# DillionLowry/NeuralCodecs

Hardware: AMD Instinct MI355X
Metric: audio-seconds/sec encode+decode (x real-time), DAC-44.1kHz B=32 (higher is better)
Workload: dtype f32; 1 GPU; DAC 44.1kHz 8kbps encode+decode, batch=32 x 1 s clips per GPU (BASELINE configs[1]); clips_per_gpu=32, global_batch=32, collective=none

## Files before the change

### neuralcodecs_amd/csrc/nc_conv_small.hip

```cpp
#include <cstdlib>
#include <type_traits>
#include <utility>
#include <vector>

#include "nc_conv.h"
#include "nc_frag.h"
#include "nc_gn.h"
#include "nc_math.h"

namespace nc {

typedef float small_f32x4 __attribute__((ext_vector_type(4)));

constexpr int SMALL_CB = 8;
constexpr int SMALL_PF = 12;

struct ConvSmallArgs {
    const float* x;
    int64_t x_bstride, x_cstride;
    int x_len;
    int in_left, in_Lz, in_L;
    const float* in_stats; const float* in_gamma; const float* in_beta; int in_elu;
    double* gn_part; int gn_nrb, gn_ncb; unsigned* gn_count; float* gn_stats; double gn_n;
    const float* wp;
    const float* bias;
    const float* alpha_out;
    float* y;
    int64_t y_bstride, y_cstride;
    int Cin, Cout, K, stride, pad, dil, Tout;
    int n_t_tiles, n_row_tiles;
    int W;
    int groups;
};

__device__ __forceinline__ float small_epilogue(const ConvSmallArgs& a, int row, float v) {
    v = v + (a.bias ? a.bias[row] : 0.0f);
    if (a.alpha_out) {
        const float al = a.alpha_out[row];
        v = nc_snakef(v, al, nc_snake_inv(al));
    }
    return v;
}

__global__ __launch_bounds__(256) void conv_small_kernel(const ConvSmallArgs a) {
    extern __shared__ __attribute__((aligned(16))) float xs[];
    const int tid = threadIdx.x, lane = tid & 63;
    const int wave = __builtin_amdgcn_readfirstlane(tid >> 6);
    int bid = blockIdx.x;
    const int rt = bid % a.n_row_tiles; bid /= a.n_row_tiles;
    const int tt = bid % a.n_t_tiles;
    const int b = bid / a.n_t_tiles;
    const int K = a.K, W = a.W, dil = a.dil;
    const int col = lane & 15, kq = lane >> 4;
    const int g0 = tt * 16 * a.stride - a.pad;
    const float* xb = a.x + (int64_t)b * a.x_bstride;
    const small_f32x4* wsrc = reinterpret_cast<const small_f32x4*>(a.wp) + ((int64_t)(4 * rt + wave) * a.groups) * 64 + lane;
    const int groups = a.groups;
    small_f32x4 ring[SMALL_PF];
#pragma unroll
    for (int i = 0; i < SMALL_PF; ++i) ring[i] = wsrc[(int64_t)min(i, groups - 1) * 64];
    const int n_blocks = (a.Cin + SMALL_CB - 1) / SMALL_CB;
    const int n_slots = SMALL_CB * W;
    constexpr int NS = 6;
    float rx[NS];
    auto issue = [&](int cbk) __attribute__((always_inline)) {
#pragma unroll
        for (int u = 0; u < NS; ++u) {
            const int i = tid + 256 * u;
            const int c = i / W, j = i - c * W;
            const int ci = cbk * SMALL_CB + c;
            int g = g0 + j;
            bool ok = (i < n_slots) & (ci < a.Cin) & (g >= 0) & (g < a.x_len);
            if (a.in_L > 0) {
                int q = g - a.in_left;
                q = q < 0 ? -q : q;
                if (q >= a.in_Lz) q = 2 * (a.in_Lz - 1) - q;
                ok = ok & (q >= 0) & (q < a.in_L);
                g = q;
            }
            rx[u] = ok ? xb[(int64_t)ci * a.x_cstride + g] : 0.0f;
        }
    };
    auto store = [&](float* dst) __attribute__((always_inline)) {
#pragma unroll
        for (int u = 0; u < NS; ++u) {
            const int i = tid + 256 * u;
            if (i < n_slots) dst[i] = rx[u];
        }
    };
    issue(0);
    store(xs);
    __syncthreads();
    small_f32x4 acc = {0.0f, 0.0f, 0.0f, 0.0f};
    const int groups_per_block = SMALL_CB * K / 16;
    int cbk = 0, gblk = 0;
    const float* xc = xs;
    if (n_blocks > 1) issue(1);
    int k = kq, off = col * a.stride + kq * dil;
    auto read_group = [&](float (&bv)[4]) __attribute__((always_inline)) {
#pragma unroll
        for (int j = 0; j < 4; ++j) {
            bv[j] = xc[off];
            k += 4; off += 4 * dil;
            if (k >= K) { k -= K; off += W - K * dil; }
        }
    };
    float bc[4], bn[4];
    read_group(bc);
    for (int gbase = 0; gbase < groups; gbase += SMALL_PF) {
        nc_static_for<SMALL_PF>([&](auto it) __attribute__((always_inline)) {
            constexpr int i = decltype(it)::value;
            if (gbase + i < groups) {
                const small_f32x4 wv = ring[i];
                ring[i] = wsrc[(int64_t)min(gbase + i + SMALL_PF, groups - 1) * 64];
                const bool last_of_block = gblk + 1 == groups_per_block;
                if (!last_of_block) read_group(bn);
#pragma unroll
                for (int j = 0; j < 4; ++j) acc = __builtin_amdgcn_mfma_f32_16x16x4f32(wv[j], bc[j], acc, 0, 0, 0);
                if (last_of_block) {
                    ++cbk;
                    gblk = 0;
                    if (cbk < n_blocks) {
                        store(xs + (cbk & 1) * n_slots);
                        __syncthreads();
                        xc = xs + (cbk & 1) * n_slots;
                        if (cbk + 1 < n_blocks) issue(cbk + 1);
                        k = kq; off = col * a.stride + kq * dil;
                        read_group(bn);
                    }
                } else {
                    ++gblk;
                }
#pragma unroll
                for (int j = 0; j < 4; ++j) bc[j] = bn[j];
            }
        });
    }
    const int t = tt * 16 + col;
    if (t < a.Tout) {
        float* yb = a.y + (int64_t)b * a.y_bstride + t;
#pragma unroll
        for (int r = 0; r < 4; ++r) {
            const int row = (4 * rt + wave) * 16 + 4 * kq + r;
            if (row < a.Cout) yb[(int64_t)row * a.y_cstride] = small_epilogue(a, row, acc[r]);
        }
    }
}

template <int GPB, int NB, int TN = 1, int CB = SMALL_CB, int NS = (TN == 1 ? 6 : TN == 2 ? 9 : 18), bool INM = false, bool GN = false>
__global__ __launch_bounds__(256) void conv_small_unrolled_kernel(const ConvSmallArgs a) {
    constexpr int BNC = 16 * TN;
    constexpr int PF = GPB * NB;
    extern __shared__ __attribute__((aligned(16))) float xs[];
    const int tid = threadIdx.x, lane = tid & 63;
    const int wave = __builtin_amdgcn_readfirstlane(tid >> 6);
    int bid = blockIdx.x;
    const int rt = bid % a.n_row_tiles; bid /= a.n_row_tiles;
    const int tt = bid % a.n_t_tiles;
    const int b = bid / a.n_t_tiles;
    const int K = a.K, W = a.W, dil = a.dil;
    const int col = lane & 15, kq = lane >> 4;
    const int g0 = tt * BNC * a.stride - a.pad;
    const float* xb = a.x + (int64_t)b * a.x_bstride;
    const small_f32x4* wsrc = reinterpret_cast<const small_f32x4*>(a.wp) + ((int64_t)(4 * rt + wave) * a.groups) * 64 + lane;
    const int groups = a.groups;
    small_f32x4 ring[PF];
#pragma unroll
    for (int i = 0; i < PF; ++i) ring[i] = wsrc[(int64_t)min(i, groups - 1) * 64];
    const int n_blocks = a.Cin / CB;
    const int n_slots = CB * W;
    float rx[NS];
    float2* const Gt = reinterpret_cast<float2*>(xs + 2 * n_slots);
    float in_mu = 0.0f, in_rs = 1.0f;
    if constexpr (INM) {
        if (a.in_stats) {
            in_mu = a.in_stats[2 * b]; in_rs = a.in_stats[2 * b + 1];
            for (int i = tid; i < a.Cin; i += 256) Gt[i] = make_float2(a.in_gamma[i], a.in_beta[i]);
        }
        __syncthreads();
    }
    int xo[NS], cu[INM ? NS : 1];
    unsigned okm = 0;
#pragma unroll
    for (int u = 0; u < NS; ++u) {
        const int i = tid + 256 * u;
        const int c = i / W, j = i - c * W;
        if constexpr (INM) cu[u] = min(c, CB - 1);
        int g = g0 + j;
        bool ok = (i < n_slots) & (g >= 0) & (g < a.x_len);
        if (a.in_L > 0) {
            int q = g - a.in_left;
            q = q < 0 ? -q : q;
            if (q >= a.in_Lz) q = 2 * (a.in_Lz - 1) - q;
            ok = ok & (q >= 0) & (q < a.in_L);
            g = q;
        }
        if (ok) okm |= 1u << u;
        xo[u] = ok ? c * (int)a.x_cstride + g : 0;
    }
    auto issue = [&](int cbk) __attribute__((always_inline)) {
        const float* xr = xb + (int64_t)cbk * CB * a.x_cstride;
#pragma unroll
        for (int u = 0; u < NS; ++u) rx[u] = xr[xo[u]];
    };
    auto store = [&](float* dst, int cbk) __attribute__((always_inline)) {
#pragma unroll
        for (int u = 0; u < NS; ++u) {
            const int i = tid + 256 * u;
            float v = rx[u];
            if constexpr (INM) {
                if (a.in_stats) {
                    const float2 gb = Gt[cbk * CB + cu[u]];
                    v = ((v - in_mu) * in_rs) * gb.x + gb.y;
                }
                if (a.in_elu) v = nc_eluf(v);
            }
            if (i < n_slots) dst[i] = ((okm >> u) & 1u) ? v : 0.0f;
        }
    };
    issue(0);
    store(xs, 0);
    __syncthreads();
    small_f32x4 acc[TN];
#pragma unroll
    for (int c = 0; c < TN; ++c) acc[c] = small_f32x4{0.0f, 0.0f, 0.0f, 0.0f};
    const int off0 = col * a.stride + kq * dil, cts = 16 * a.stride;
    for (int cb0 = 0; cb0 < n_blocks; cb0 += NB) {
        nc_static_for<NB>([&](auto bt) __attribute__((always_inline)) {
            constexpr int nb = decltype(bt)::value;
            const int cbk = cb0 + nb;
            const float* xc = xs + (cbk & 1) * n_slots;
            const int nxt = min(cbk + 1, n_blocks - 1);
            issue(nxt);
            int k = kq, off = off0;
            if constexpr (CB == 64) { k = 0; off = col * a.stride + kq * W; }
            else if (k >= K) { k -= K; off += W - K * dil; }
            float bv[2][4][TN];
            auto read_group = [&](float (&v)[4][TN]) __attribute__((always_inline)) {
#pragma unroll
                for (int j = 0; j < 4; ++j) {
#pragma unroll
                    for (int c = 0; c < TN; ++c) v[j][c] = xc[off + c * cts];
                    if constexpr (CB == 64) {
                        off += 4 * W;
                    } else {
                        k += 4; off += 4 * dil;
                        if (k >= K) { k -= K; off += W - K * dil; }
                        if (k >= K) { k -= K; off += W - K * dil; }
                    }
                }
            };
            read_group(bv[0]);
            nc_static_for<GPB>([&](auto gt) __attribute__((always_inline)) {
                constexpr int g = decltype(gt)::value, ri = nb * GPB + g;
                const small_f32x4 wv = ring[ri];
                ring[ri] = wsrc[(int64_t)min((cbk + NB) * GPB + g, groups - 1) * 64];
                if constexpr (g + 1 < GPB) read_group(bv[(g + 1) & 1]);
#pragma unroll
                for (int j = 0; j < 4; ++j)
#pragma unroll
                    for (int c = 0; c < TN; ++c) acc[c] = __builtin_amdgcn_mfma_f32_16x16x4f32(wv[j], bv[g & 1][j][c], acc[c], 0, 0, 0);
            });
            store(xs + ((cbk + 1) & 1) * n_slots, nxt);
            __syncthreads();
        });
    }
    if constexpr (GN) {
        static_assert(!GN || TN == 2, "the GroupNorm epilogue reduces whole 32x32 blocks: 32-column tiles");
        float* const tile = xs;
#pragma unroll
        for (int c = 0; c < TN; ++c)
#pragma unroll
            for (int r = 0; r < 4; ++r) {
                const int lr = 16 * wave + 4 * kq + r, row = 64 * rt + lr;
                tile[lr * 33 + c * 16 + col] = acc[c][r] + ((a.bias && row < a.Cout) ? a.bias[row] : 0.0f);
            }
        __syncthreads();
        if (wave < 2) {
            const int h = lane >> 5, cc = lane & 31;
            const int t = tt * 32 + cc;
            float vv[16];
            unsigned okm16 = 0;
#pragma unroll
            for (int r = 0; r < 16; ++r) {
                const int lr = 32 * wave + (r & 3) + 8 * (r >> 2) + 4 * h;
                vv[r] = tile[lr * 33 + cc];
                if ((64 * rt + lr < a.Cout) & (t < a.Tout)) okm16 |= 1u << r;
            }
            double s1, s2;
            nc_gn_slot_sums<false>(vv, okm16, s1, s2);
            nc_gn_butterfly(s1, s2);
            const int rbk = 2 * rt + wave, cbk = tt;
            if (lane == 0 && rbk < a.gn_nrb && cbk < a.gn_ncb)
                nc_gn_store_partial(a.gn_part + (((int64_t)b * a.gn_nrb + rbk) * a.gn_ncb + cbk) * 2, s1, s2);
        }
        if (a.gn_count != nullptr)
            nc_gn_arrive_and_finish(a.gn_part + (int64_t)b * a.gn_nrb * a.gn_ncb * 2, a.gn_count + b, a.gn_stats + 2 * b, a.gn_nrb * a.gn_ncb,
                                    (unsigned)(a.n_row_tiles * a.n_t_tiles), a.gn_n);
    }
#pragma unroll
    for (int c = 0; c < TN; ++c) {
        const int t = tt * BNC + c * 16 + col;
        if (t < a.Tout) {
            float* yb = a.y + (int64_t)b * a.y_bstride + t;
#pragma unroll
            for (int r = 0; r < 4; ++r) {
                const int row = (4 * rt + wave) * 16 + 4 * kq + r;
                if (row < a.Cout) yb[(int64_t)row * a.y_cstride] = small_epilogue(a, row, acc[c][r]);
            }
        }
    }
}

void pack_conv_small(const float* dense_w, int Cin, int Cout, int K, std::vector<float>& out) {
    const int tiles = ((Cout + 63) / 64) * 4, groups = Cin * K / 16;
    out.assign((size_t)tiles * groups * 256, 0.0f);
    for (int tile = 0; tile < tiles; ++tile)
        for (int g = 0; g < groups; ++g)
            for (int l = 0; l < 64; ++l)
                for (int j = 0; j < 4; ++j) {
                    const int row = 16 * tile + (l & 15), kk = 16 * g + 4 * j + (l >> 4);
                    if (row < Cout) out[(((size_t)tile * groups + g) * 64 + l) * 4 + j] = dense_w[(size_t)row * Cin * K + kk];
                }
}

static bool small_k1(int Cin, int Cout, int K, int stride) { return K == 1 && stride == 1 && Cin % 256 == 0 && Cout >= 1024; }
static bool small_k7(int Cin, int K, int stride, int dil) { return (K == 7 || K == 3) && stride == 1 && dil == 1 && Cin % 32 == 0; }

bool conv_small_eligible(int Cin, int Cout, int K, int stride, int dil, bool transposed) {
    if (!transposed && small_k1(Cin, Cout, K, stride)) return true;
    if (!transposed && Cout >= 64 && small_k7(Cin, K, stride, dil)) return true;
    if (transposed || K < 4 || stride < 2 || Cout < 64) return false;
    if ((Cin * K) % 16 != 0 || (SMALL_CB * K) % 16 != 0 || Cin % SMALL_CB != 0) return false;
    const int W = 15 * stride + (K - 1) * dil + 1;
    return SMALL_CB * W <= 6 * 256 && (size_t)2 * SMALL_CB * W * 4 <= 64 * 1024;
}

int conv_small_max_tn(int Cin, int K, int stride, int dil) {
    if (K == 1 && stride == 1 && Cin % 256 == 0) return 2;
    if (small_k7(Cin, K, stride, dil)) return 2;
    const int W32 = 31 * stride + (K - 1) * dil + 1;
    const bool k16 = K * SMALL_CB / 16 == 8 && Cin % SMALL_CB == 0 && (Cin / SMALL_CB) % 2 == 0;
    return (k16 && SMALL_CB * W32 <= 9 * 256) ? 2 : 1;
}

bool conv_small_gn_available(int Cin, int K, int stride, int dil, bool inm) {
    if (conv_small_max_tn(Cin, K, stride, dil) < 2) return false;
    if (small_k7(Cin, K, stride, dil)) return K == 3 ? Cin <= 1024 : !inm;
    return !inm;
}

bool conv_small_inm_available(int Cin, int K, int stride, int dil) { return K == 3 && small_k7(Cin, K, stride, dil) && Cin <= 1024; }

bool launch_conv_small(const float* x, int64_t x_bstride, int64_t x_cstride, int x_len, int in_left, int in_Lz, int in_L, const float* in_stats,
                       const float* in_gamma, const float* in_beta, int in_elu, const ConvSmallGn* gn, const float* wp, const float* bias, const float* alpha_out, float* y,
                       int64_t y_bstride, int64_t y_cstride, int B, int Cin, int Cout, int K, int stride, int pad, int dil, int Tout, int want_tn, hipStream_t s) {
    ConvSmallArgs a{};
    a.x = x; a.x_bstride = x_bstride; a.x_cstride = x_cstride; a.x_len = x_len; a.wp = wp; a.bias = bias; a.alpha_out = alpha_out;
    a.in_left = in_left; a.in_Lz = in_Lz; a.in_L = in_L;
    a.in_stats = in_stats; a.in_gamma = in_gamma; a.in_beta = in_beta; a.in_elu = in_elu;
    if (gn && gn->part) {
        if (alpha_out || conv_small_max_tn(Cin, K, stride, dil) < 2) return false;
        a.gn_part = gn->part; a.gn_nrb = gn->nrb; a.gn_ncb = gn->ncb; a.gn_count = gn->count; a.gn_stats = gn->stats; a.gn_n = gn->n;
        want_tn = 2;
    }
    const bool with_gn = a.gn_part != nullptr;
    const bool inm = in_stats != nullptr || in_elu != 0;
    if (inm && !conv_small_inm_available(Cin, K, stride, dil)) return false;
    a.y = y; a.y_bstride = y_bstride; a.y_cstride = y_cstride;
    a.Cin = Cin; a.Cout = Cout; a.K = K; a.stride = stride; a.pad = pad; a.dil = dil; a.Tout = Tout;
    a.n_row_tiles = (Cout + 63) / 64;
    a.groups = Cin * K / 16;
    static const int tn_env = (int)env_int("NC_SMALL_TN", 0);
    const int W64 = 63 * stride + (K - 1) * dil + 1;
    const bool tn2_fits = conv_small_max_tn(Cin, K, stride, dil) >= 2, tn4_fits = tn2_fits && SMALL_CB * W64 <= 18 * 256;
    const int TN = with_gn ? 2 : (tn4_fits && tn_env == 4 && !small_k7(Cin, K, stride, dil)) ? 4 : (tn2_fits && (tn_env == 2 || (tn_env == 0 && want_tn >= 2))) ? 2 : 1;
    a.n_t_tiles = (Tout + 16 * TN - 1) / (16 * TN);
    a.W = (16 * TN - 1) * stride + (K - 1) * dil + 1;
    const bool k7 = small_k7(Cin, K, stride, dil), k1 = small_k1(Cin, Cout, K, stride);
    size_t lds = (size_t)2 * (k1 ? 64 : k7 ? 16 : SMALL_CB) * a.W * sizeof(float) + (inm ? (size_t)Cin * sizeof(float2) : 0);
    if (with_gn) lds = std::max(lds, (size_t)64 * 33 * sizeof(float));
    const int64_t grid = (int64_t)B * a.n_t_tiles * a.n_row_tiles;
    if (grid <= 0 || grid > 0x7fffffff) return false;
    static const bool rolled_only = env_flag("NC_SMALL_ROLLED");
    const int gpb = SMALL_CB * K / 16, n_blocks = Cin / SMALL_CB;
    const bool fits31 = (int64_t)Cin * x_cstride + x_len < ((int64_t)1 << 31);
    void (*fn)(const ConvSmallArgs) = conv_small_kernel;
    if (k1) {
        if (!fits31 || TN != 2 || with_gn || inm) return false;
        fn = conv_small_unrolled_kernel<4, 4, 2, 64, 8>;
    } else if (k7) {
        if (!fits31) return false;
        if (with_gn) {
            if (K == 7 && !inm) fn = conv_small_unrolled_kernel<7, 2, 2, 16, 3, false, true>;
            else if (K == 3) fn = conv_small_unrolled_kernel<3, 2, 2, 16, 3, true, true>;
            else return false;
        } else if (K == 7) fn = TN == 2 ? conv_small_unrolled_kernel<7, 2, 2, 16, 3> : conv_small_unrolled_kernel<7, 2, 1, 16, 2>;
        else if (inm) fn = TN == 2 ? conv_small_unrolled_kernel<3, 2, 2, 16, 3, true> : conv_small_unrolled_kernel<3, 2, 1, 16, 2, true>;
        else fn = TN == 2 ? conv_small_unrolled_kernel<3, 2, 2, 16, 3> : conv_small_unrolled_kernel<3, 2, 1, 16, 2>;
    } else if (TN == 4) {
        if (!fits31) return false;
        fn = conv_small_unrolled_kernel<8, 2, 4>;
    } else if (TN == 2) {
        if (!fits31 || (with_gn && inm)) return false;
        fn = with_gn ? conv_small_unrolled_kernel<8, 2, 2, SMALL_CB, 9, false, true> : conv_small_unrolled_kernel<8, 2, 2>;
    } else if (!rolled_only && fits31 && Cin % SMALL_CB == 0) {
        if (gpb == 8 && n_blocks % 2 == 0) fn = conv_small_unrolled_kernel<8, 2>;
        else if (gpb == 4 && n_blocks % 4 == 0) fn = conv_small_unrolled_kernel<4, 4>;
        else if (gpb == 5 && n_blocks % 4 == 0) fn = conv_small_unrolled_kernel<5, 4>;
        else if (gpb == 3 && n_blocks % 6 == 0) fn = conv_small_unrolled_kernel<3, 6>;
        else if (gpb == 2 && n_blocks % 8 == 0) fn = conv_small_unrolled_kernel<2, 8>;
    }
    hipLaunchKernelGGL(fn, dim3((unsigned)grid), dim3(256), lds, s, a);
    NC_HIP(hipGetLastError());
    return true;
}

}
```

### neuralcodecs_amd/csrc/nc_util.hip

```cpp
#include <cmath>
#include <mutex>
#include <set>
#include <tuple>

#include "nc_common.h"
#include "nc_model.h"

namespace nc {

static thread_local std::string g_last_error;
void set_last_error(const char* msg) { g_last_error = msg ? msg : ""; }
const char* get_last_error() { return g_last_error.c_str(); }

namespace {
struct EnvRow { const char* name; char kind; const char* doc; };
const EnvRow kEnv[] = {
    {"NC_NO_FLAT", 'b', "one-clip column tiles instead of the flattened (clip, column) axis"},
    {"NC_NO_FLAT_GN", 'b', "one-clip tiles wherever GroupNorm sums are emitted"},
    {"NC_CO_GROUP", 'i', "cap of the row-tile groups (1 = one weight panel per XCD)"},
    {"NC_NO_WIDE_FUSE", 'b', "no whole-channel fused residual units (C = 256)"},
    {"NC_WIDE_FUSE_192", 'b', "whole-channel fused unit at C = 192 as well"},
    {"NC_NO_FUSE", 'b', "every residual unit in two launches"},
    {"NC_NO_TILE_ALTS", 'b', "primary row-tile height only"},
    {"NC_TM_PICK", 'i', "force a packed row-tile variant"},
    {"NC_TM_FORCE", 'i', "force the row-tile height where it divides Cout"},
    {"NC_TN_THRESH", 'i', "column-tile width threshold"},
    {"NC_NO_TN_ROUNDS", 'b', "no round-count rule for the column-tile width"},
    {"NC_NO_XR", 'b', "generic B-fragment addressing in the conv template (no constant-pitch immediate offsets)"},
    {"NC_NO_XV", 'b', "legacy instances with item-wise window staging everywhere (no XV-only instances)"},
    {"NC_XV_K7_MIN_COLS", 'i', "columns per clip from which the k = 7 convolutions take the XV-only instances (0: wherever the rows are 64-byte aligned)"},
    {"NC_NO_XV_K7", 'b', "legacy instances for the k = 7 residual-unit convolutions (no XV-only instances on the long rows)"},
    {"NC_NO_NARROW", 'b', "no 3-wave narrow variants"},
    {"NC_NO_SLIM", 'b', "no half-size reduction blocks for narrow long rows"},
    {"NC_NO_SUBPIXEL", 'b', "per-phase launches for power-of-two strided transposed convolutions"},
    {"NC_NO_SUBPIXEL_ANY", 'b', "per-phase launches for the other strides (3, 5)"},
    {"NC_NO_CONV1X1", 'b', "pointwise layers through the windowed template"},
    {"NC_NO_SKINNY", 'b', "no skinny projection kernel (Cout <= 16)"},
    {"NC_NO_THIN", 'b', "PCM heads through the matrix-core template"},
    {"NC_THIN_NO_VEC", 'p', "scalar window loads in the thin-output kernel"},
    {"NC_NO_THIN_INM", 'b', "summed copy + plain head instead of the input-mode head"},
    {"NC_NO_STEM", 'b', "stems through the matrix-core template"},
    {"NC_NO_TINY_TILES", 'b', "no smallest-tile rule for tiny grids"},
    {"NC_TINY_BLOCKS", 'i', "grid size below which the tiny-grid rule applies (256)"},
    {"NC_NO_DIST_SMALL", 'b', "segmented staging on small grids"},
    {"NC_DIST_MAX_GRID", 'i', "largest grid that takes distributed staging (768)"},
    {"NC_NO_CONV_SMALL", 'b', "no short-row 16x16x4 kernel"},
    {"NC_SMALL_MAX_GRID", 'i', "largest short-row grid (2048)"},
    {"NC_SMALL_WIDE_BELOW", 'i', "template grid below which the 32-column short-row form is taken (512)"},
    {"NC_SMALL_K1_COLS", 'i', "columns up to which k = 1 layers take the short-row kernel (4096; 0 = off)"},
    {"NC_SMALL_TN", 'i', "force the short-row column tiles (1 | 2 | 4)"},
    {"NC_SMALL_ROLLED", 'b', "rolled short-row loop"},
    {"NC_DAC_RVQ_STAGEWISE", 'p', "DAC quantizer stage by stage"},
    {"NC_EUCLID_NO_MFMA", 'p', "vector Euclidean codebook search"},
    {"NC_ENCODEC_NO_FUSE", 'b', "padded / activated copies instead of the fused SConv1d input mode"},
    {"NC_ENCODEC_NO_OVERLAP", 'b', "segment groups one after the other"},
    {"NC_NO_GN_FUSE", 'b', "stand-alone GroupNorm sums"},
    {"NC_NO_GN_FINISH", 'b', "separate GroupNorm final launch"},
    {"NC_NO_IN2", 'b', "summed copies instead of the two-input staging mode"},
    {"NC_NO_CONV3S", 'b', "windowed k = 3 instead of the streaming kernel"},
    {"NC_DAC_PITCH", 'b', "DAC activation rows at pitch L rounded up to 16 samples (64-byte aligned rows: the 696-step layers take the XV-only instances; measured slower)"},
    {"NC_NO_DOWN2", 'b', "Encodec 48 kHz encoder: the windowed two-input instance for the stride-2 down-convolution instead of the streaming kernel"},
    {"NC_NO_DOWN4", 'b', "Encodec 48 kHz encoder: summed copy + windowed instance for the stride-4 down-convolution instead of the streaming kernel"},
    {"NC_NO_DOWN5", 'b', "Encodec 48 kHz encoder: summed copy + windowed instance for the stride-5 down-convolution instead of the streaming kernel"},
    {"NC_NO_UP_PITCH", 'b', "Encodec transposed convolutions write dense rows (the trimmed view of the stride-5 layer then starts on an odd sample)"},
    {"NC_NO_UP4", 'b', "Encodec 48 kHz decoder: summed copy + windowed instance for the stride-4 up-convolution instead of the streaming kernel"},
    {"NC_NO_UP2", 'b', "Encodec 48 kHz decoder: the windowed two-input instance for the stride-2 up-convolution instead of the streaming kernel"},
    {"NC_RMS_TWO_PASS", 'b', "Encodec RMS scale as two launches (chunk sums, final) instead of the one-launch form"},
    {"NC_NO_RES_A", 'b', "residual blocks of the Encodec 48 kHz outer stages: shortcut and k = 3 branch as two launches instead of the fused first pass"},
    {"NC_SYNC_ACQUIRE", 'b', "agent-scope acquire fence behind the persistent LSTM's flag poll and in front of the in-launch GroupNorm finish"},
    {"NC_LSTM_STEPWISE", 'b', "one LSTM launch per step"},
    {"NC_LSTM_CHUNKS", 'i', "layer-pipeline chunks of the per-layer persistent LSTM (6; 1 = layers in sequence)"},
    {"NC_LSTM_EVEN_CHUNKS", 'b', "equal LSTM chunks"},
    {"NC_LSTM_UB", 'i', "hidden-unit blocks per LSTM workgroup (2 | 4)"},
    {"NC_LSTM_NO_HTILE", 'b', "persistent LSTM: every wavefront fetches its own h operands, W_hh in LDS (the form before the LDS h tile)"},
    {"NC_LSTM_NO_ELU", 'b', "the consumer applies the ELU behind an SLSTM"},
    {"NC_LSTM_FAKE_TIMEOUT", 'b', "tests: report the first persistent LSTM launch as timed out"},
    {"NC_SNAC_NO_FUSE", 'b', "SNAC residual units in two launches (depthwise, pointwise)"},
    {"NC_SNAC_FUSE_MIN_COLS", 'i', "columns (clips x steps) from which the one-launch SNAC residual unit is taken (65536)"},
    {"NC_SNAC_FUSE_MAX_ELEMS", 'i', "channels x steps of ONE clip up to which the one-launch SNAC residual unit is taken (2^30: its 32-bit lane offsets; tests lower it)"},
    {"NC_SNAC_UNIT_TRACE", 's', "file for the in-kernel stamps of the first one-launch SNAC residual unit at C = 96"},
    {"NC_DW_NO_VEC", 'b', "scalar depthwise kernel"},
    {"NC_LN_TILE", 'i', "LayerNorm tile width (8 | 16; 0 = one thread per column)"},
    {"NC_ATTN_NO_MFMA", 'b', "vector local-attention kernel"},
    {"NC_RCCL_LIB", 's', "the one RCCL library to open"},
    {"NC_LAUNCH_LOG", 's', "launch log for the per-class PMC attribution"},
    {"NC_CONV_TRACE_FILE", 's', "-DNC_CONV_TRACE builds: file for the in-kernel phase trace of the convolution template (tools/probe/conv_trace.py)"},
    {"NC_CONV_TRACE_SEL", 's', "-DNC_CONV_TRACE builds: \"K,Cin,dilation\" of the launch to trace (default 7,384,1)"},
};
const EnvRow& env_row(const char* name, char kind) {
    for (const EnvRow& r : kEnv)
        if (std::strcmp(r.name, name) == 0) {
            if (r.kind != kind) fail(NC_ESTATE, "switch %s is registered as kind '%c', read as '%c'", name, r.kind, kind);
            return r;
        }
    fail(NC_ESTATE, "switch %s is not in the table of nc_util.hip", name);
}
}
bool env_flag(const char* name) { const char* v = std::getenv(env_row(name, 'b').name); return v && v[0] == '1'; }
bool env_present(const char* name) { return std::getenv(env_row(name, 'p').name) != nullptr; }
long env_int(const char* name, long dflt) { const char* v = std::getenv(env_row(name, 'i').name); return v ? atol(v) : dflt; }
const char* env_str(const char* name) { const char* v = std::getenv(env_row(name, 's').name); return v && v[0] ? v : nullptr; }
FILE* launch_log() {
    static FILE* lf = [] { const char* p = env_str("NC_LAUNCH_LOG"); return p ? std::fopen(p, "w") : (FILE*)nullptr; }();
    return lf;
}
const char* env_switch_table() {
    static const std::string text = [] {
        std::string t;
        for (const EnvRow& r : kEnv) { t += r.name; t += '\t'; t += r.kind; t += '\t'; t += r.doc; t += '\n'; }
        return t;
    }();
    return text.c_str();
}

void ensure_dynamic_lds(const void* fn, size_t bytes) {
    static std::mutex mu;
    static std::set<std::tuple<int, const void*, size_t>> done;
    int dev = 0;
    NC_HIP(hipGetDevice(&dev));
    std::lock_guard<std::mutex> g(mu);
    const auto key = std::make_tuple(dev, fn, bytes);
    if (done.count(key)) return;
    NC_HIP(hipFuncSetAttribute(fn, hipFuncAttributeMaxDynamicSharedMemorySize, (int)bytes));
    done.insert(key);
}

void Blob::parse(const void* data, size_t nbytes) {
    const uint8_t* buf = static_cast<const uint8_t*>(data);
    if (!buf || nbytes < 24 || std::memcmp(buf, "NCWB0001", 8) != 0) fail(NC_EINVAL, "not an NCWB0001 weight blob");
    storage.assign(buf, buf + nbytes);
    buf = storage.data();
    uint64_t n, idx_len;
    std::memcpy(&n, buf + 8, 8);
    std::memcpy(&idx_len, buf + 16, 8);
    if (idx_len > nbytes - 24) fail(NC_EINVAL, "weight blob index exceeds the image");
    const uint64_t data0 = (24 + idx_len + 63) & ~uint64_t(63);
    if (data0 > nbytes) fail(NC_EINVAL, "weight blob index exceeds the image");
    const uint64_t idx_end = 24 + idx_len;
    uint64_t p = 24;
    tensors.clear();
    auto need = [&](uint64_t k) {
        if (k > idx_end - p) fail(NC_EINVAL, "truncated weight blob index");
    };
    for (uint64_t i = 0; i < n; ++i) {
        need(2);
        uint16_t ln;
        std::memcpy(&ln, buf + p, 2);
        p += 2;
        need((uint64_t)ln + 2);
        BlobTensor t;
        t.name.assign(reinterpret_cast<const char*>(buf + p), ln);
        p += ln;
        t.dtype = buf[p];
        const int nd = buf[p + 1];
        p += 2;
        if (t.dtype != 0 && t.dtype != 1) fail(NC_EINVAL, "tensor %s: unknown dtype %d (0 = float32, 1 = int64)", t.name.c_str(), t.dtype);
        if (nd > 8) fail(NC_EINVAL, "tensor %s has %d dimensions (at most 8)", t.name.c_str(), nd);
        need((uint64_t)nd * 8 + 16);
        uint64_t numel = 1;
        for (int d = 0; d < nd; ++d) {
            uint64_t v;
            std::memcpy(&v, buf + p, 8);
            p += 8;
            if (v > (uint64_t)1 << 40 || (v != 0 && numel > ((uint64_t)1 << 40) / v)) fail(NC_EINVAL, "tensor %s: dimensions overflow", t.name.c_str());
            numel *= v;
            t.dims.push_back((int64_t)v);
        }
        uint64_t off, nb;
        std::memcpy(&off, buf + p, 8);
        std::memcpy(&nb, buf + p + 8, 8);
        p += 16;
        const uint64_t room = nbytes - data0;
        if (off > room || nb > room - off) fail(NC_EINVAL, "tensor %s exceeds the weight blob", t.name.c_str());
        if (nb != numel * (t.dtype == 0 ? 4 : 8))
            fail(NC_EINVAL, "tensor %s: %llu bytes for %llu elements of dtype %d", t.name.c_str(), (unsigned long long)nb, (unsigned long long)numel, t.dtype);
        t.data = buf + data0 + off;
        t.nbytes = (int64_t)nb;
        tensors[t.name] = t;
    }
}

const BlobTensor* Blob::find(const std::string& name) const {
    auto it = tensors.find(name);
    if (it == tensors.end()) return nullptr;
    if (it->second.dtype != 0) fail(NC_EINVAL, "weight tensor '%s' is not float32", name.c_str());
    return &it->second;
}

const BlobTensor& Blob::get(const std::string& name) const {
    const BlobTensor* t = find(name);
    if (!t) fail(NC_ENOTFOUND, "weight tensor '%s' not found in blob", name.c_str());
    return *t;
}

void fold_weight_norm_dac(const float* v, const float* g, int64_t d0, int64_t inner, float* w) {
    for (int64_t i = 0; i < d0; ++i) {
        double ss = 0.0;
        for (int64_t j = 0; j < inner; ++j) {
            const float q = v[i * inner + j] * v[i * inner + j];
            ss += (double)q;
        }
        const float denom = std::sqrt((float)ss) + 1e-7f;
        for (int64_t j = 0; j < inner; ++j) w[i * inner + j] = (v[i * inner + j] / denom) * g[i];
    }
}

hipEvent_t Profiler::get_event() {
    if (!pool.empty()) {
        hipEvent_t e = pool.back();
        pool.pop_back();
        return e;
    }
    hipEvent_t e;
    NC_HIP(hipEventCreate(&e));
    return e;
}

void Profiler::begin(hipStream_t s, int cls, double flops, double bytes) {
    Pending pd{get_event(), get_event(), cls, flops, bytes};
    NC_HIP(hipEventRecord(pd.a, s));
    pending.push_back(pd);
}

void Profiler::end(hipStream_t s) { NC_HIP(hipEventRecord(pending.back().b, s)); }

void Profiler::resolve() {
    for (auto& pd : pending) {
        NC_HIP(hipEventSynchronize(pd.b));
        float ms = 0.f;
        NC_HIP(hipEventElapsedTime(&ms, pd.a, pd.b));
        acc[pd.cls].launches += 1;
        acc[pd.cls].ms += ms;
        acc[pd.cls].flops += pd.flops;
        acc[pd.cls].bytes += pd.bytes;
        pool.push_back(pd.a);
        pool.push_back(pd.b);
    }
    pending.clear();
}

void Profiler::reset() {
    resolve();
    for (auto& e : acc) e = nc_profile_entry{};
}

Profiler::~Profiler() {
    for (auto& pd : pending) {
        (void)hipEventDestroy(pd.a);
        (void)hipEventDestroy(pd.b);
    }
    for (auto e : pool) (void)hipEventDestroy(e);
}

__global__ void copy_rows_kernel(const uint32_t* __restrict__ src, int64_t spitch_w, uint32_t* __restrict__ dst, int64_t dpitch_w, int64_t width_w,
                                 int64_t rows) {
    const int64_t i = (int64_t)blockIdx.x * 256 + threadIdx.x;
    if (i >= rows * width_w) return;
    const int64_t r = i / width_w, c = i - r * width_w;
    dst[r * dpitch_w + c] = src[r * spitch_w + c];
}

void launch_copy_rows(void* dst, size_t dpitch, const void* src, size_t spitch, size_t width, size_t rows, hipStream_t s) {
    if (!width || !rows) return;
    if ((dpitch | spitch | width) & 3 || width > dpitch || width > spitch) fail(NC_ESTATE, "internal: pitched copy of %zu bytes per row (pitches %zu, %zu)", width, spitch, dpitch);
    const int64_t n = (int64_t)rows * (int64_t)(width / 4), grid = (n + 255) / 256;
    if (grid > 0x7fffffff) fail(NC_EUNSUPPORTED, "pitched copy of %lld words exceeds one grid", (long long)n);
    hipLaunchKernelGGL(copy_rows_kernel, dim3((unsigned)grid), dim3(256), 0, s, static_cast<const uint32_t*>(src), (int64_t)(spitch / 4),
                       static_cast<uint32_t*>(dst), (int64_t)(dpitch / 4), (int64_t)(width / 4), (int64_t)rows);
    NC_HIP(hipGetLastError());
}

}
```

Baseline: 596.8 audio-seconds/sec.

## Add batched short-row conv kernel with 64/96 columns per weight fragment

```diff
diff --git a/neuralcodecs_amd/csrc/nc_conv_small.hip b/neuralcodecs_amd/csrc/nc_conv_small.hip
--- a/neuralcodecs_amd/csrc/nc_conv_small.hip
+++ b/neuralcodecs_amd/csrc/nc_conv_small.hip
@@ -312,6 +312,154 @@
     }
 }
 
+constexpr int small_batched_q(int K, int S, int TN) {
+    const int q = ((16 * TN - 1) * S + K + S - 1) / S;
+    return q + ((16 - q % 32) + 32) % 32;
+}
+constexpr int small_batched_pitch(int K, int S, int TN) {
+    if (S > 1) return S * small_batched_q(K, S, TN);
+    const int w = 16 * TN - 1 + K;
+    return w + (((K + 15) % 32 - w % 32) + 32) % 32;
+}
+constexpr int small_batched_slot(int n, int K, int S, int TN) {
+    const int c = n / K, k = n % K;
+    return c * small_batched_pitch(K, S, TN) + (S > 1 ? (k % S) * small_batched_q(K, S, TN) + k / S : k);
+}
+
+template <int K, int S, int TN, int CB, int PFD>
+__global__ __launch_bounds__(256, 2) void conv_small_batched_kernel(const ConvSmallArgs a) {
+    static_assert(S == 1 || S == 8, "stride 1 (position-major window) or stride 8 (phase-major, the staging permutation is 8 x 8)");
+    static_assert(K % 4 == 0 || S == 1, "a tap count that splits lane groups over channel rows: stride 1 only");
+    static_assert(CB % 4 == 0 && (CB * K) % 16 == 0, "whole channels per wave, whole groups per block");
+    constexpr int BNC = 16 * TN, GPB = CB * K / 16, STEPS = 4 * GPB;
+    static_assert((2 * GPB) % PFD == 0, "ring positions are compile-time constants over a two-block iteration");
+    constexpr int W = (BNC - 1) * S + K;
+    constexpr int Q = S > 1 ? small_batched_q(K, S, TN) : 1, WP = small_batched_pitch(K, S, TN);
+    constexpr int CPW = CB / 4, NV = (W + 63) / 64, VS = 64 / S;
+    static_assert(S == 1 || NV * 64 <= WP, "every staged position has a slot");
+    extern __shared__ __attribute__((aligned(16))) float xs[];
+    const int tid = threadIdx.x, lane = tid & 63;
+    const int wave = __builtin_amdgcn_readfirstlane(tid >> 6);
+    int bid = blockIdx.x;
+    const int rt = bid % a.n_row_tiles; bid /= a.n_row_tiles;
+    const int tt = bid % a.n_t_tiles;
+    const int b = bid / a.n_t_tiles;
+    const int col = lane & 15, kq = lane >> 4;
+    const int g0 = tt * BNC * S - a.pad;
+    const float* xb = a.x + (int64_t)b * a.x_bstride;
+    const small_f32x4* wsrc = reinterpret_cast<const small_f32x4*>(a.wp) + ((int64_t)(4 * rt + wave) * a.groups) * 64 + lane;
+    const int groups = a.groups;
+    small_f32x4 ring[PFD];
+#pragma unroll
+    for (int i = 0; i < PFD; ++i) ring[i] = wsrc[(int64_t)min(i, groups - 1) * 64];
+    const int n_blocks = a.Cin / CB;
+    const int jl = S > 1 ? (lane & 7) * 8 + (lane >> 3) : lane;
+    const int sbase = wave * CPW * WP + (S > 1 ? (jl & 7) * Q + (jl >> 3) : jl);
+    unsigned pj[NV];
+    unsigned okm = 0;
+#pragma unroll
+    for (int v = 0; v < NV; ++v) {
+        const int j = jl + 64 * v, g = g0 + j;
+        const bool ok = (j < W) & (g >= 0) & (g < a.x_len);
+        if (ok) okm |= 1u << v;
+        pj[v] = ok ? 4u * (unsigned)g : 0u;
+    }
+    float rx[CPW][NV];
+    auto issue = [&](int cbk) __attribute__((always_inline)) {
+#pragma unroll
+        for (int cc = 0; cc < CPW; ++cc) {
+            const char* xr = reinterpret_cast<const char*>(xb + (int64_t)(cbk * CB + wave * CPW + cc) * a.x_cstride);
+#pragma unroll
+            for (int v = 0; v < NV; ++v) rx[cc][v] = *reinterpret_cast<const float*>(xr + pj[v]);
+        }
+    };
+    auto store = [&](float* dst) __attribute__((always_inline)) {
+#pragma unroll
+        for (int cc = 0; cc < CPW; ++cc)
+#pragma unroll
+            for (int v = 0; v < NV; ++v)
+                if (64 * v + 63 < W || jl + 64 * v < W) dst[sbase + cc * WP + v * VS] = ((okm >> v) & 1u) ? rx[cc][v] : 0.0f;
+    };
+    issue(0);
+    store(xs);
+    __syncthreads();
+    small_f32x4 acc[TN];
+#pragma unroll
+    for (int c = 0; c < TN; ++c) acc[c] = small_f32x4{0.0f, 0.0f, 0.0f, 0.0f};
+    const int lane_base = col + kq * Q;
+    int offs[K % 4 == 0 ? 1 : STEPS];
+    if constexpr (K % 4 != 0) {
+#pragma unroll
+        for (int st = 0; st < STEPS; ++st) {
+            const int n = 4 * st + kq, c = n / K;
+            offs[st] = c * WP + (n - c * K) + col;
+        }
+    }
+    for (int cb0 = 0; cb0 < n_blocks; cb0 += 2) {
+        nc_static_for<2>([&](auto bt) __attribute__((always_inline)) {
+            constexpr int nb = decltype(bt)::value;
+            const int cbk = cb0 + nb;
+            const float* xc = xs + nb * (CB * WP);
+            const int nxt = min(cbk + 1, n_blocks - 1);
+            issue(nxt);
+            __builtin_amdgcn_sched_barrier(0);
+            float bv[2][TN];
+            auto read_step = [&](auto sc, float (&v)[TN]) __attribute__((always_inline)) {
+                constexpr int st = decltype(sc)::value;
+#pragma unroll
+                for (int c = 0; c < TN; ++c) {
+                    if constexpr (K % 4 == 0) v[c] = xc[lane_base + small_batched_slot(4 * st, K, S, TN) + 16 * c];
+                    else v[c] = xc[offs[st] + 16 * c];
+                }
+            };
+            read_step(std::integral_constant<int, 0>{}, bv[0]);
+            nc_static_for<STEPS>([&](auto sc) __attribute__((always_inline)) {
+                constexpr int st = decltype(sc)::value, g = st / 4, j = st % 4, slot = (nb * GPB + g) % PFD;
+                if constexpr (st + 1 < STEPS) read_step(std::integral_constant<int, st + 1>{}, bv[(st + 1) & 1]);
+#pragma unroll
+                for (int c = 0; c < TN; ++c) acc[c] = __builtin_amdgcn_mfma_f32_16x16x4f32(ring[slot][j], bv[st & 1][c], acc[c], 0, 0, 0);
+                if constexpr (j == 3) {
+                    ring[slot] = wsrc[(int64_t)min(cbk * GPB + g + PFD, groups - 1) * 64];
+                    __builtin_amdgcn_sched_barrier(0);
+                }
+            });
+            store(xs + (1 - nb) * (CB * WP));
+            __syncthreads();
+        });
+    }
+#pragma unroll
+    for (int c = 0; c < TN; ++c) {
+        const int t = tt * BNC + c * 16 + col;
+        if (t < a.Tout) {
+            float* yb = a.y + (int64_t)b * a.y_bstride + t;
+#pragma unroll
+            for (int r = 0; r < 4; ++r) {
+                const int row = (4 * rt + wave) * 16 + 4 * kq + r;
+                if (row < a.Cout) yb[(int64_t)row * a.y_cstride] = small_epilogue(a, row, acc[c][r]);
+            }
+        }
+    }
+}
+
+typedef void (*conv_small_fn)(const ConvSmallArgs);
+static conv_small_fn small_batched_instance(int K, int stride, int Cin, int TN, size_t* lds) {
+    if (TN != 4 && TN != 6) return nullptr;
+    const bool t6 = TN == 6;
+    if (K == 16 && stride == 8 && Cin % 16 == 0) {
+        *lds = (size_t)2 * 8 * small_batched_pitch(16, 8, TN) * sizeof(float);
+        return t6 ? conv_small_batched_kernel<16, 8, 6, 8, 8> : conv_small_batched_kernel<16, 8, 4, 8, 8>;
+    }
+    if (K == 7 && stride == 1 && Cin % 32 == 0) {
+        *lds = (size_t)2 * 16 * small_batched_pitch(7, 1, TN) * sizeof(float);
+        return t6 ? conv_small_batched_kernel<7, 1, 6, 16, 7> : conv_small_batched_kernel<7, 1, 4, 16, 7>;
+    }
+    if (K == 3 && stride == 1 && Cin % 32 == 0) {
+        *lds = (size_t)2 * 16 * small_batched_pitch(3, 1, TN) * sizeof(float);
+        return t6 ? conv_small_batched_kernel<3, 1, 6, 16, 6> : conv_small_batched_kernel<3, 1, 4, 16, 6>;
+    }
+    return nullptr;
+}
+
 void pack_conv_small(const float* dense_w, int Cin, int Cout, int K, std::vector<float>& out) {
     const int tiles = ((Cout + 63) / 64) * 4, groups = Cin * K / 16;
     out.assign((size_t)tiles * groups * 256, 0.0f);
@@ -351,6 +499,14 @@
 }
 
 bool conv_small_inm_available(int Cin, int K, int stride, int dil) { return K == 3 && small_k7(Cin, K, stride, dil) && Cin <= 1024; }
+
+static void log_small_form(conv_small_fn fn, int64_t grid, size_t lds, hipStream_t s) {
+    if (FILE* lf = launch_log()) {
+        const char* sym = hipKernelNameRefByPtr((const void*)fn, s);
+        std::fprintf(lf, "small_form %s %lld %zu\n", sym ? sym : "?", (long long)grid, lds);
+        std::fflush(lf);
+    }
+}
 
 bool launch_conv_small(const float* x, int64_t x_bstride, int64_t x_cstride, int x_len, int in_left, int in_Lz, int in_L, const float* in_stats,
                        const float* in_gamma, const float* in_beta, int in_elu, const ConvSmallGn* gn, const float* wp, const float* bias, const float* alpha_out, float* y,
@@ -375,6 +531,24 @@
     const int W64 = 63 * stride + (K - 1) * dil + 1;
     const bool tn2_fits = conv_small_max_tn(Cin, K, stride, dil) >= 2, tn4_fits = tn2_fits && SMALL_CB * W64 <= 18 * 256;
     const int TN = with_gn ? 2 : (tn4_fits && tn_env == 4 && !small_k7(Cin, K, stride, dil)) ? 4 : (tn2_fits && (tn_env == 2 || (tn_env == 0 && want_tn >= 2))) ? 2 : 1;
+    static const int64_t batched_min_grid = env_int("NC_SMALL_BATCHED_MIN_GRID", 1024);
+    static const bool no_batched = env_flag("NC_SMALL_NO_BATCHED");
+    if (TN == 2 && tn_env == 0 && !no_batched && !with_gn && !inm && in_L == 0 && dil == 1 && x_len > 0 && x_len < (1 << 30) &&
+        (int64_t)B * ((Tout + 31) / 32) * a.n_row_tiles >= batched_min_grid) {
+        const int cols32 = (Tout + 31) / 32 * 32;
+        for (const int btn : {6, 4}) {
+            const int tiles = (Tout + 16 * btn - 1) / (16 * btn);
+            size_t blds = 0;
+            const conv_small_fn bfn = tiles * 16 * btn <= cols32 ? small_batched_instance(K, stride, Cin, btn, &blds) : nullptr;
+            const int64_t bgrid = (int64_t)B * tiles * a.n_row_tiles;
+            if (!bfn || bgrid > 0x7fffffff) continue;
+            a.n_t_tiles = tiles;
+            hipLaunchKernelGGL(bfn, dim3((unsigned)bgrid), dim3(256), blds, s, a);
+            NC_HIP(hipGetLastError());
+            log_small_form(bfn, bgrid, blds, s);
+            return true;
+        }
+    }
     a.n_t_tiles = (Tout + 16 * TN - 1) / (16 * TN);
     a.W = (16 * TN - 1) * stride + (K - 1) * dil + 1;
     const bool k7 = small_k7(Cin, K, stride, dil), k1 = small_k1(Cin, Cout, K, stride);
@@ -413,6 +587,7 @@
     }
     hipLaunchKernelGGL(fn, dim3((unsigned)grid), dim3(256), lds, s, a);
     NC_HIP(hipGetLastError());
+    log_small_form(fn, grid, lds, s);
     return true;
 }
 
diff --git a/neuralcodecs_amd/csrc/nc_util.hip b/neuralcodecs_amd/csrc/nc_util.hip
--- a/neuralcodecs_amd/csrc/nc_util.hip
+++ b/neuralcodecs_amd/csrc/nc_util.hip
@@ -50,6 +50,8 @@
     {"NC_SMALL_K1_COLS", 'i', "columns up to which k = 1 layers take the short-row kernel (4096; 0 = off)"},
     {"NC_SMALL_TN", 'i', "force the short-row column tiles (1 | 2 | 4)"},
     {"NC_SMALL_ROLLED", 'b', "rolled short-row loop"},
+    {"NC_SMALL_BATCHED_MIN_GRID", 'i', "32-column short-row grid from which the batched form (64 / 96 columns per weight fragment) is taken (1024)"},
+    {"NC_SMALL_NO_BATCHED", 'b', "no batched short-row form: the 32-column instances on the many-clip launches as well"},
     {"NC_DAC_RVQ_STAGEWISE", 'p', "DAC quantizer stage by stage"},
     {"NC_EUCLID_NO_MFMA", 'p', "vector Euclidean codebook search"},
     {"NC_ENCODEC_NO_FUSE", 'b', "padded / activated copies instead of the fused SConv1d input mode"},
```

After: 601.7 audio-seconds/sec (median of 6 runs). Within noise of the previous version (+0.8%).
